# hukenovs/blackman_harris_win

Measured on AMD Instinct MI355X. Metric: window Gsamples/s (BH-7, N=2^26, 32-bit) + fraction of HBM-write roofline, higher is better.
Workload: dtype int64

## Files before the change

### blackman_harris_win_amd/csrc/bhw_build.hip

```cpp
#include "bhw_device.h"

namespace {

template <typename T>
__global__ __launch_bounds__(kBlock) void k_table_build(BhwCordicCfg cfg, uint32_t entries, void *__restrict__ table)
{
    __shared__ T lut_s[32];
    stage_lut<T>(cfg, lut_s);
    const uint32_t u = blockIdx.x * kBlock + threadIdx.x;
    if (u >= entries) return;
    T x, y;
    cordic_q1<T>(lut_s, (T)cfg.x0, (T)((T)u << cfg.z_shl), (int)cfg.n_iter, x, y);
    const int32_t c = (int32_t)(x >> cfg.out_shr), sn = (int32_t)(y >> cfg.out_shr);
    const int2 head = make_int2(__builtin_amdgcn_readfirstlane(c), __builtin_amdgcn_readfirstlane(sn));
    const int4 rec = cfg.tab_dlog > kPackLog ? reinterpret_cast<const int4 *>(cfg.tab_coarse)[u >> fmt_cell_log(cfg.tab_dlog)] : make_int4(0, 0, 0, 0);
    tab_store(table, u, cfg.phi_width - 2 - cfg.z_shr, cfg.tab_split, cfg.tab_dlog, const_cast<void *>(cfg.tab_coarse), c, sn, head, rec,
              cfg.tab_check);
}


template <int NITER, int FMT>
__global__ __launch_bounds__(kBuildThreads) void k_table_build_shared(BhwBuildPlan plan, void *__restrict__ table)
{
    __shared__ int64_t gx[kGroupsPerWg];
    __shared__ int64_t gy[kGroupsPerWg];
    __shared__ int32_t gz[kGroupsPerWg];
    __shared__ int32_t gk[kGroupsPerWg];
    __shared__ uint32_t lut_s[32];
    if (threadIdx.x < 32) lut_s[threadIdx.x] = plan.lut[threadIdx.x];
    __syncthreads();

    constexpr int n_iter = NITER;
    const uint32_t s = plan.z_shl;
    const uint32_t gpw = plan.groups_per_wg;
    const uint32_t group0 = blockIdx.x * gpw;
    const uint32_t n_groups = plan.entries >> 6;

    if (threadIdx.x < gpw) {
        const uint32_t g = group0 + threadIdx.x;
        const uint32_t u_first = g << 6;
        int64_t x = plan.x0, y = plan.x0;
        int32_t zf = (int32_t)((u_first << s) - lut_s[0]);
        const uint32_t span = 63u << s;
        int k = 1;
        bool live = g < n_groups;
        constexpr int kmax = n_iter < kPrefixMax ? n_iter : kPrefixMax;
#pragma unroll
        for (int kk = 1; kk < kmax; ++kk) {
            if (live) {
                const int32_t zl = (int32_t)((uint32_t)zf + span);
                if ((zf < 0) != (zl < 0)) {
                    live = false;
                } else {
                    rot_step(x, y, zf, kk, plan.lut[kk]);
                    k = kk + 1;
                }
            }
        }
        gx[threadIdx.x] = x;
        gy[threadIdx.x] = y;
        gz[threadIdx.x] = zf;
        gk[threadIdx.x] = k;
    }
    __syncthreads();

    const uint32_t wave = __builtin_amdgcn_readfirstlane(threadIdx.x >> 6), lane = threadIdx.x & 63u;
    uint32_t idx_a = lane, idx_m = 64u;
    if (plan.tab_split) {
        const uint32_t e = 1u << plan.log2_entries;
        if (lane & 1u)      { idx_a = (e >> 1) + (lane >> 1); idx_m = 32u; }
        else if (lane & 2u) { idx_a = (e >> 2) + (lane >> 2); idx_m = 16u; }
        else                { idx_a = lane >> 2;              idx_m = 16u; }
    }
    for (uint32_t gi = wave; gi < gpw; gi += kBuildThreads / 64) {
        const uint32_t g = __builtin_amdgcn_readfirstlane(group0 + gi);
        if (g >= n_groups) break;
        int64_t x = gx[gi], y = gy[gi];
        int32_t z = (int32_t)((uint32_t)gz[gi] + (lane << s));
        const int k0 = __builtin_amdgcn_readfirstlane(gk[gi]);
#pragma unroll
        for (int k = 1; k < NITER; ++k) {
            if (k >= kPrefixMax || k >= k0) rot_step(x, y, z, k, plan.lut[k]);
        }
        const int32_t c = (int32_t)(x >> plan.out_shr), sn = (int32_t)(y >> plan.out_shr);
        const int2 head = make_int2(__builtin_amdgcn_readfirstlane(c), __builtin_amdgcn_readfirstlane(sn));
        const uint32_t idx = idx_a + g * idx_m;
        if constexpr (FMT == 4) {
            const uint32_t u = (g << 6) + lane, nmask = 4u * plan.entries - 1u;
            int32_t *d_sin = reinterpret_cast<int32_t *>(table), *d_cos = reinterpret_cast<int32_t *>(const_cast<void *>(plan.tab_coarse));
#pragma unroll
            for (uint32_t q = 0; q < 4u; ++q) {
                int32_t oc, os;
                quadrant_map(q, c, sn, plan.pad0, oc, os);
                const uint32_t i = (q * plan.entries + u - plan.pad) & nmask;
                if (d_sin) d_sin[i] = os;
                if (d_cos) d_cos[i] = oc;
            }
        } else if constexpr (FMT == 0) {
            reinterpret_cast<int2 *>(table)[idx] = make_int2(c, sn);
        } else {
            static_assert(FMT == 1, "k_table_build_shared builds plain and delta16 tables (and the sin / cos sweep) only");
            const int32_t dc = c - head.x, ds = sn - head.y;
            if (plan.check_flag && !(fits_bits(dc, 16) && fits_bits(ds, 16))) atomicOr(plan.check_flag, 1u);
            reinterpret_cast<uint32_t *>(table)[idx] = ((uint32_t)dc & 0xFFFFu) | ((uint32_t)ds << 16);
            if (lane == 0u) reinterpret_cast<int2 *>(const_cast<void *>(plan.tab_coarse))[g] = head;
        }
    }
}

constexpr int kMirrorTail = 6;
constexpr int mirror_gpw(int threads) { return threads / 4; }
constexpr int mirror_heads_max(int threads) { return mirror_gpw(threads) / 2 + 8; }
constexpr int mirror_heads_pad(int threads) { return (mirror_heads_max(threads) + 63) / 64 * 64; }
constexpr int kTailZ = 256;

constexpr int kTailRows = 65;
struct TailD { int8_t v[kTailRows * 64 + 16]; };
constexpr TailD make_tail_d()
{
    TailD t{};
    for (int p = 0; p < 64; ++p)
        for (int v = 0; v < kTailRows; ++v) {
            int d = 0;
            for (int j = 0; j < kMirrorTail; ++j) d += ((p >> j) & 1) ? -(v >> j) : (v >> j);
            t.v[v * 64 + p] = (int8_t)d;
        }
    return t;
}
__device__ const TailD kTailD = make_tail_d();

constexpr int kRankSkip = 4;
constexpr int kRankCand = (1 << kRankSkip) + 1;
template <typename L>
__device__ __forceinline__ int32_t rank_threshold(uint32_t p, const L &l)
{
    int32_t t = 0;
#pragma unroll
    for (int m = 0; m + 1 < kRankSkip; ++m) {
        const uint32_t bit = 1u << (kRankSkip - 1 - m);
        if (p & (bit - 1u)) t += (p & bit) ? (int32_t)l[m] : -(int32_t)l[m];
    }
    return t;
}
template <int M, int R>
__device__ __forceinline__ void rank_candidates(uint32_t x, uint32_t y, uint32_t k, uint32_t bk, uint2 *out)
{
    if constexpr (M == kRankSkip) out[R] = make_uint2(x, y);
    else {
        const uint32_t a = y >> k, b = (x >> k) + bk;
        rank_candidates<M + 1, 2 * R>(x + a, y - b, k + 1u, bk >> 1, out);
        rank_candidates<M + 1, 2 * R + 1>(x - a, y + b, k + 1u, bk >> 1, out);
    }
}

template <int K, bool ZERO>
__device__ __forceinline__ void rot_narrow(uint32_t &x, uint32_t &y, int32_t &z, uint32_t &zacc, uint32_t lutk)
{
    uint32_t a, b;
    if constexpr (ZERO) {
        asm volatile("v_lshrrev_b32 %[a], %[k], %[y]\n\t"
                     "v_lshrrev_b32 %[b], %[k], %[x]\n\t"
                     "v_min_u32 %[za], %[za], %[z]\n\t"
                     "v_cmpx_gt_i32 vcc, 0, %[z]\n\t"
                     "v_add_u32 %[x], %[x], %[a]\n\t"
                     "v_sub_u32 %[y], %[y], %[b]\n\t"
                     "v_add_u32 %[z], %[z], %[l]\n\t"
                     "s_not_b64 exec, exec\n\t"
                     "v_sub_u32 %[x], %[x], %[a]\n\t"
                     "v_add_u32 %[y], %[y], %[b]\n\t"
                     "v_sub_u32 %[z], %[z], %[l]\n\t"
                     "s_mov_b64 exec, -1"
                     : [x] "+v"(x), [y] "+v"(y), [z] "+v"(z), [za] "+v"(zacc), [a] "=&v"(a), [b] "=&v"(b)
                     : [l] "s"(lutk), [k] "n"(K)
                     : "vcc", "scc");
    } else {
        asm volatile("v_lshrrev_b32 %[a], %[k], %[y]\n\t"
                     "v_lshrrev_b32 %[b], %[k], %[x]\n\t"
                     "v_cmpx_gt_i32 vcc, 0, %[z]\n\t"
                     "v_add_u32 %[x], %[x], %[a]\n\t"
                     "v_sub_u32 %[y], %[y], %[b]\n\t"
                     "v_add_u32 %[z], %[z], %[l]\n\t"
                     "s_not_b64 exec, exec\n\t"
                     "v_sub_u32 %[x], %[x], %[a]\n\t"
                     "v_add_u32 %[y], %[y], %[b]\n\t"
                     "v_sub_u32 %[z], %[z], %[l]\n\t"
                     "s_mov_b64 exec, -1"
                     : [x] "+v"(x), [y] "+v"(y), [z] "+v"(z), [a] "=&v"(a), [b] "=&v"(b)
                     : [l] "s"(lutk), [k] "n"(K)
                     : "vcc", "scc");
    }
}

template <int KA, int NITER>
__device__ __forceinline__ void rot_narrow_block(uint32_t &x, uint32_t &y, int32_t &z, uint32_t &zacc, const uint32_t (&l)[10], int e, uint32_t hi)
{
    uint32_t a, b;
#define BHW_ROT_I(lbl, i, HI_ADD)                                                                                       \
    #lbl ":\n\t"                                                                                                        \
    "v_lshrrev_b32 %[a], %[k" #i "], %[y]\n\t"                                                                          \
    "v_lshrrev_b32 %[b], %[k" #i "], %[x]\n\t"                                                                          \
    HI_ADD                                                                                                             \
    "v_min_u32 %[za], %[za], %[z]\n\t"                                                                                  \
    "v_cmpx_gt_i32 vcc, 0, %[z]\n\t"                                                                                    \
    "v_add_u32 %[x], %[x], %[a]\n\t"                                                                                    \
    "v_sub_u32 %[y], %[y], %[b]\n\t"                                                                                    \
    "v_add_u32 %[z], %[z], %[l" #i "]\n\t"                                                                              \
    "s_not_b64 exec, exec\n\t"                                                                                          \
    "v_sub_u32 %[x], %[x], %[a]\n\t"                                                                                    \
    "v_add_u32 %[y], %[y], %[b]\n\t"                                                                                    \
    "v_sub_u32 %[z], %[z], %[l" #i "]\n\t"                                                                              \
    "s_mov_b64 exec, -1\n"
#define BHW_ROT_PLAIN(i) BHW_ROT_I(i, i, "")
#define BHW_ROT_HI(i) BHW_ROT_I(2##i, i, "v_add_u32 %[b], %[c" #i "], %[b]\n\t")
#define BHW_ROT_DISPATCH(P, H)                                                                                         \
                 "s_cmp_gt_i32 %[e], 4\n\ts_cbranch_scc1 " #H "f\n\t"                                                 \
                 "s_cmp_lt_i32 %[e], 1\n\ts_cbranch_scc1 " #P "0f\n\t"                                                 \
                 "s_cmp_eq_u32 %[e], 1\n\ts_cbranch_scc1 " #P "1f\n\t"                                                 \
                 "s_cmp_eq_u32 %[e], 2\n\ts_cbranch_scc1 " #P "2f\n\t"                                                 \
                 "s_cmp_eq_u32 %[e], 3\n\ts_cbranch_scc1 " #P "3f\n\t"                                                 \
                 "s_branch " #P "4f\n"                                                                                  \
                 #H ":\n\t"                                                                                            \
                 "s_cmp_eq_u32 %[e], 5\n\ts_cbranch_scc1 " #P "5f\n\t"                                                 \
                 "s_cmp_eq_u32 %[e], 6\n\ts_cbranch_scc1 " #P "6f\n\t"                                                 \
                 "s_cmp_eq_u32 %[e], 7\n\ts_cbranch_scc1 " #P "7f\n\t"                                                 \
                 "s_cmp_eq_u32 %[e], 8\n\ts_cbranch_scc1 " #P "8f\n\t"                                                 \
                 "s_cmp_eq_u32 %[e], 9\n\ts_cbranch_scc1 " #P "9f\n\t"
    constexpr int S = NITER - 1 - KA;
    static_assert(S >= 9 && S <= 30, "bias shifts");
    asm volatile("s_cmp_lg_u32 %[hi], 0\n\ts_cbranch_scc1 100f\n\t"
                 BHW_ROT_DISPATCH(, 40)
                 "s_branch 10f\n"
                 BHW_ROT_PLAIN(0) BHW_ROT_PLAIN(1) BHW_ROT_PLAIN(2) BHW_ROT_PLAIN(3) BHW_ROT_PLAIN(4) BHW_ROT_PLAIN(5) BHW_ROT_PLAIN(6) BHW_ROT_PLAIN(7)
                 BHW_ROT_PLAIN(8) BHW_ROT_PLAIN(9)
                 "10:\n\ts_branch 200f\n"
                 "100:\n\t"
                 BHW_ROT_DISPATCH(2, 41)
                 "s_branch 200f\n"
                 BHW_ROT_HI(0) BHW_ROT_HI(1) BHW_ROT_HI(2) BHW_ROT_HI(3) BHW_ROT_HI(4) BHW_ROT_HI(5) BHW_ROT_HI(6) BHW_ROT_HI(7) BHW_ROT_HI(8) BHW_ROT_HI(9)
                 "200:"
                 : [x] "+v"(x), [y] "+v"(y), [z] "+v"(z), [za] "+v"(zacc), [a] "=&v"(a), [b] "=&v"(b)
                 : [e] "s"(e), [hi] "s"(hi), [l0] "s"(l[0]), [l1] "s"(l[1]), [l2] "s"(l[2]), [l3] "s"(l[3]), [l4] "s"(l[4]),
                   [l5] "s"(l[5]), [l6] "s"(l[6]), [l7] "s"(l[7]), [l8] "s"(l[8]), [l9] "s"(l[9]),
                   [k0] "n"(KA), [k1] "n"(KA + 1), [k2] "n"(KA + 2), [k3] "n"(KA + 3), [k4] "n"(KA + 4), [k5] "n"(KA + 5), [k6] "n"(KA + 6),
                   [k7] "n"(KA + 7), [k8] "n"(KA + 8), [k9] "n"(KA + 9),
                   [c0] "n"(1 << S), [c1] "n"(1 << (S - 1)), [c2] "n"(1 << (S - 2)), [c3] "n"(1 << (S - 3)), [c4] "n"(1 << (S - 4)),
                   [c5] "n"(1 << (S - 5)), [c6] "n"(1 << (S - 6)), [c7] "n"(1 << (S - 7)), [c8] "n"(1 << (S - 8)), [c9] "n"(1 << (S - 9))
                 : "vcc", "scc");
#undef BHW_ROT_I
#undef BHW_ROT_PLAIN
#undef BHW_ROT_HI
#undef BHW_ROT_DISPATCH
}

#ifdef BHW_BUILD_STAMPS
__device__ unsigned long long *g_build_stamps = nullptr;
#define BHW_STAMP(i) do { if (g_build_stamps && (threadIdx.x & 63u) == 0u) atomicMax(&g_build_stamps[blockIdx.x * 16u + (i)], (unsigned long long)wall_clock64()); } while (0)
#define BHW_STAMP_MIN(i) do { if (g_build_stamps && threadIdx.x == 0u) g_build_stamps[blockIdx.x * 16u + (i)] = (unsigned long long)wall_clock64(); } while (0)
#else
#define BHW_STAMP(i) do { } while (0)
#define BHW_STAMP_MIN(i) do { } while (0)
#endif

template <int BYTES>
__device__ __forceinline__ void table_store(void *__restrict__ table, uint32_t idx, uint32_t v)
{
    if constexpr (BYTES == 1) asm volatile("global_store_byte %0, %1, %2 sc1" :: "v"(idx), "v"(v), "s"(table) : "memory");
    else asm volatile("global_store_short %0, %1, %2 sc1" :: "v"(idx << 1), "v"(v), "s"(table) : "memory");
}

template <int NITER, int FMT, int THREADS>
__global__ __launch_bounds__(THREADS) __attribute__((amdgpu_waves_per_eu(8, 8))) void k_table_build_mirror(BhwBuildPlan plan, void *__restrict__ table)
{
    BHW_STAMP_MIN(0);
#ifdef BHW_BUILD_STAMPS
    if (g_build_stamps && threadIdx.x == 0u) {
        uint32_t hw, xcc;
        asm volatile("s_getreg_b32 %0, hwreg(HW_REG_HW_ID)\n\ts_getreg_b32 %1, hwreg(HW_REG_XCC_ID)" : "=s"(hw), "=s"(xcc));
        g_build_stamps[blockIdx.x * 16u + 6u] = hw;
        g_build_stamps[blockIdx.x * 16u + 7u] = xcc;
    }
#endif
    static_assert(FMT == 2 || FMT == 3 || FMT == 5, "residual / nibble entries");
    static_assert(NITER >= 21 && NITER <= 32, "narrow state: 32-bit words");
    static_assert(THREADS == 256 || THREADS == 1024, "workgroup shapes");
    constexpr uint32_t gpw = mirror_gpw(THREADS);
    constexpr uint32_t kHeads = mirror_heads_max(THREADS), kHeadsPad = mirror_heads_pad(THREADS);
    static_assert(gpw + 2 * kHeadsPad + 64 <= THREADS, "prefix lanes, two ranges of head chains, the tail-table wave");
    __shared__ int4 gst[gpw];
    __shared__ int2 ghi[gpw];
    __shared__ uint32_t lut_s[32];
    __shared__ uint8_t tail_p[2 * kTailZ];
    __shared__ __attribute__((aligned(16))) int8_t tail_d[kTailRows * 64 + 16];
    constexpr bool kRank = THREADS == 1024 || FMT != 5;
    __shared__ uint2 cand_s[kRank ? gpw * kRankCand : 1];
    __shared__ int2 rank_tab[kRank ? 8 << kRankSkip : 1];
    constexpr uint32_t kWorkMax = 8 * gpw;
    __shared__ uint32_t work_n;
    __shared__ uint32_t work_u[kWorkMax];
    __shared__ uint32_t esc_n;
    __shared__ int4 esc_list[FMT == 5 ? kEscFill : 1];
    __shared__ int4 esc_tab[FMT == 5 ? kEscSlots : 1];
    if (threadIdx.x < 32) lut_s[threadIdx.x] = plan.lut[threadIdx.x];
    if constexpr (FMT == 5) {
        if (threadIdx.x >= 64u && threadIdx.x < 64u + kEscSlots) esc_tab[threadIdx.x - 64u] = make_int4(-1, 0, 0, 0);
    }
#ifdef BHW_BUILD_STAMPS
    if (g_build_stamps && threadIdx.x == 0u) { asm volatile("s_waitcnt lgkmcnt(0)" ::: "memory"); g_build_stamps[blockIdx.x * 16u + 8u] = (unsigned long long)wall_clock64() | (plan.entries & 0u); }
#endif
    constexpr int n_iter = NITER;
    constexpr int KS = NITER - kMirrorTail;
    constexpr int KA = KS - 10;
    constexpr int kRankTop = KS - kRankSkip < kPrefixMax ? KS - kRankSkip : kPrefixMax;
    static_assert(kRankTop - KA < 8 && kRankTop + kRankSkip <= 31, "rank_tab rows; ROM words");
    const uint32_t s = plan.z_shl;
    const uint32_t group0 = blockIdx.x * gpw;
    const uint32_t E = plan.entries;
    const uint32_t n_groups = E >> 7;
    const uint32_t u_lo = group0 << 6;
    const uint32_t u_hi = ((group0 + gpw) << 6) < (n_groups << 6) ? ((group0 + gpw) << 6) : (n_groups << 6);
    const uint32_t m_last = (E >> 1) - 1u;
    if (threadIdx.x == 0) {
        work_n = 0u;
        esc_n = 0u;
        if (u_hi == (E >> 1)) {
            work_u[0] = E >> 1;
            work_n = 1u;
        }
    }
    if (threadIdx.x >= (uint32_t)THREADS - 64u) {
        const uint32_t t3 = threadIdx.x - ((uint32_t)THREADS - 64u);
#pragma unroll
        for (int q = 0; q < 5; ++q)
            if (t3 + 64u * q < (uint32_t)(kTailRows * 64 + 16) / 16u) reinterpret_cast<int4 *>(tail_d)[t3 + 64u * q] = reinterpret_cast<const int4 *>(kTailD.v)[t3 + 64u * q];
#pragma unroll
        for (int q = 0; q < 2 * kTailZ / 64; ++q) {
            const uint32_t zi = t3 + 64u * (uint32_t)q;
            int32_t z = (int32_t)zi - kTailZ;
            uint32_t p = 0u;
#pragma unroll
            for (int j = 0; j < kMirrorTail; ++j) {
                if (z < 0) { p |= 1u << j; z += (int32_t)plan.lut[KS + j]; } else z -= (int32_t)plan.lut[KS + j];
            }
            tail_p[zi] = (uint8_t)p;
        }
        if (kRank && t3 < (1u << kRankSkip)) {
#pragma unroll
            for (int row = 0; row <= kRankTop - KA; ++row) {
                const uint32_t l[kRankSkip] = {plan.lut[KA + row], plan.lut[KA + row + 1], plan.lut[KA + row + 2], plan.lut[KA + row + 3]};
                int32_t off = 0;
#pragma unroll
                for (int m = 0; m < kRankSkip; ++m) off += (t3 >> (kRankSkip - 1 - m)) & 1u ? (int32_t)l[m] : -(int32_t)l[m];
                rank_tab[(row << kRankSkip) + t3] = make_int2(off, t3 ? rank_threshold(t3, l) : INT32_MIN);
            }
        }
        BHW_STAMP(9);
    }


    __shared__ int32_t hc[2][kHeads], hs[2][kHeads];
    const uint32_t d = fmt_cell_log(plan.tab_dlog);
    const uint32_t cells_total = E >> d;
    uint32_t cell_lo[2] = {0u, 0u}, n_cell[2] = {0u, 0u}, r_lo[2] = {u_lo, 0u}, r_hi[2] = {u_hi, 0u};
    {
        const uint32_t a = u_lo > 1u ? u_lo : 1u, b = (u_hi - 1u) < m_last ? (u_hi - 1u) : m_last;
        if (a <= b) { r_lo[1] = E - b; r_hi[1] = E - a + 1u; }
        if (a <= b && b == (E >> 1) - 1u) r_lo[1] = E >> 1;
    }
#pragma unroll
    for (int w = 0; w < 2; ++w)
        if (r_hi[w] > r_lo[w]) {
            cell_lo[w] = r_lo[w] >> d;
            n_cell[w] = ((r_hi[w] - 1u) >> d) - cell_lo[w] + 1u;
        }
    if (threadIdx.x >= gpw && threadIdx.x < gpw + 2u * kHeadsPad) {
        const uint32_t w = (threadIdx.x - gpw) / kHeadsPad;
        const uint32_t t = (threadIdx.x - gpw) % kHeadsPad;
        if (n_cell[w] && t < n_cell[w] + 2u) {
            const int64_t cell = (t <= n_cell[w]) ? (int64_t)cell_lo[w] + t : (int64_t)cell_lo[w] - 1;
            if (cell >= 0 && cell < (int64_t)cells_total) {
                int64_t x = plan.x0, y = plan.x0;
                int32_t z = (int32_t)((((uint32_t)cell << d) << s) - plan.lut[0]);
#pragma unroll
                for (int r = 1; r < n_iter; ++r) rot_step(x, y, z, r, plan.lut[r]);
                hc[w][t] = (int32_t)(x >> plan.out_shr);
                hs[w][t] = (int32_t)(y >> plan.out_shr);
            }
        }
        BHW_STAMP(10);
    }

    constexpr int kcap = KS < kPrefixMax ? KS : kPrefixMax;
    if (threadIdx.x < gpw) {
        const uint32_t g = group0 + threadIdx.x;
        const uint32_t u_first = g << 6;
        int64_t x = plan.x0, y = plan.x0;
        int32_t zf = (int32_t)((u_first << s) - plan.lut[0]);
        const uint32_t span = 63u << s;
        int k = 1;
        bool live = g < n_groups;
        uint32_t zero0 = 0u;
#pragma unroll
        for (int kk = 1; kk < kcap; ++kk) {
            if (live) {
                const int32_t zl = (int32_t)((uint32_t)zf + span);
                if ((zf < 0) != (zl < 0)) {
                    live = false;
                } else {
                    zero0 |= (uint32_t)(zf == 0);
                    rot_step(x, y, zf, kk, plan.lut[kk]);
                    k = kk + 1;
                }
            }
        }
        const int64_t drift = ((int64_t)1 << (NITER - k + 1)) + 2, lim = (int64_t)1 << NITER;
        const bool narrow = x >= drift && y >= drift && x + drift < lim && y + drift < lim;
        constexpr int64_t kBias = (int64_t)1 << (NITER - 1);
        const bool hi = !narrow && k >= KS - 10 && y >= drift && y + drift < lim && x - kBias >= drift && x - kBias + drift < ((int64_t)1 << 32) &&
                        x + drift < lim + ((int64_t)1 << KS);
        const int64_t xp = hi ? x - kBias : x;
        uint32_t flags = zero0 | (narrow || hi ? 2u : 0u) | (hi ? 4u : 0u) | (g == 0u ? 8u : 0u);
        uint32_t w0 = (uint32_t)xp, w1 = (uint32_t)y, kw = (uint32_t)k;
        if (kRank && (narrow || hi) && k >= KA && k <= kRankTop) {
            uint32_t l[kRankSkip - 1] = {};
#pragma unroll
            for (int kk = KA; kk <= kRankTop; ++kk)
                if (k == kk) {
#pragma unroll
                    for (int m = 0; m + 1 < kRankSkip; ++m) l[m] = plan.lut[kk + m];
                }
            uint64_t mask = 0ull;
            uint32_t below = 0u, above = 0u;
            bool ok = true;
            int32_t prev = INT32_MIN;
            const int32_t round_up = (int32_t)((1u << s) - 1u) - zf;
#pragma unroll
            for (uint32_t p = 1; p < (1u << kRankSkip); ++p) {
                const int32_t t = rank_threshold(p, l);
                ok = ok && t > prev;
                prev = t;
                const int32_t first = (t + round_up) >> s;
                if (first <= 0) ++below;
                else if (first > 63) ++above;
                else mask |= 1ull << (first - 1);
            }
            if (ok && (uint32_t)__builtin_popcountll(mask) + below + above == (1u << kRankSkip) - 1u) {
                rank_candidates<0, 0>((uint32_t)xp, (uint32_t)y, (uint32_t)k, hi ? 1u << (NITER - 1 - k) : 0u, &cand_s[threadIdx.x * kRankCand]);
                w0 = (uint32_t)mask;
                w1 = (uint32_t)(mask >> 32);
                kw = (uint32_t)(k + kRankSkip) | (below << 16) | ((uint32_t)(k - KA) << (20 + kRankSkip + 3));
                flags |= 16u;
            }
        }
        gst[threadIdx.x] = make_int4((int32_t)w0, (int32_t)w1, zf, (int32_t)(kw | (flags << 8)));
        ghi[threadIdx.x] = make_int2((int32_t)(xp >> 32), (int32_t)(y >> 32));
        BHW_STAMP(11);
    }
    BHW_STAMP(1);
    __syncthreads();

    __shared__ int4 hrec[2][kHeads];
    {
        const uint32_t w = threadIdx.x / kHeadsPad, t = threadIdx.x % kHeadsPad;
        if (w < 2u && t < n_cell[w]) {
            const uint32_t cell = cell_lo[w] + t;
            int4 r;
            if (cell + 1u < cells_total) r = make_int4(hc[w][t], hs[w][t], hc[w][t + 1] - hc[w][t], hs[w][t + 1] - hs[w][t]);
            else {
                const uint32_t tp = t ? t - 1u : n_cell[w] + 1u;
                r = make_int4(hc[w][t], hs[w][t], hc[w][t] - hc[w][tp], hs[w][t] - hs[w][tp]);
            }
            if constexpr (FMT == 5) { r.x += (int32_t)kEscBias; r.y += (int32_t)kEscBias; }
            if constexpr (fmt_is_nibble(FMT)) { r.x -= 8; r.y -= 8; }
            hrec[w][t] = r;
            if constexpr (fmt_is_nibble(FMT)) { r.z *= 2; r.w *= 2; }
            if ((cell << d) >= r_lo[w])
                reinterpret_cast<int4 *>(const_cast<void *>(plan.tab_coarse))[cell] = r;
        }
    }
    __syncthreads();
    BHW_STAMP_MIN(2);
    auto record_of = [&](int w, uint32_t cell) -> int4 { return hrec[w][cell - cell_lo[w]]; };

    auto store_entry = [&](auto CHECKED, uint32_t idx, int32_t c, int32_t sn, const int4 rec, uint32_t pos) {
        if constexpr (FMT == 5) {
            const int2 p = tab_predict(rec, pos, d);
            const uint32_t nc = (uint32_t)(c - p.x), ns = (uint32_t)(sn - p.y);
            uint32_t v = nc | (ns << 4);
            if (__builtin_expect((int)(nc - 1u > 14u) | (int)(ns > 15u), 0)) {
                const uint32_t slot = atomicAdd(&esc_n, 1u);
                if (slot < kEscFill) esc_list[slot] = make_int4((int32_t)idx, c, sn, 0);
                v = kEscMarker;
            }
            table_store<1>(table, idx, v);
        } else if constexpr (FMT == 3) {
            const int2 p = tab_predict(rec, pos, d);
            const uint32_t nc = (uint32_t)(c - p.x), ns = (uint32_t)(sn - p.y);
            if constexpr (decltype(CHECKED)::value) {
                if (plan.check_flag && (nc | ns) > 15u) atomicOr(plan.check_flag, 1u);
            }
            table_store<1>(table, idx, nc | (ns << 4));
        } else {
            const int2 p = tab_predict(rec, pos, d);
            const int32_t dc = c - p.x, ds = sn - p.y;
            if constexpr (decltype(CHECKED)::value) {
                if (plan.check_flag && !(fits_bits(dc, 8) && fits_bits(ds, 8))) atomicOr(plan.check_flag, 1u);
            }
            table_store<2>(table, idx, ((uint32_t)dc & 0xFFu) | ((uint32_t)ds << 8));
        }
    };

    const uint32_t wave = __builtin_amdgcn_readfirstlane(threadIdx.x >> 6), lane = threadIdx.x & 63u;
    uint32_t idx_a, idx_m, idx_i;
    if (lane & 1u)      { idx_a = (E >> 1) + (lane >> 1); idx_m = 32u; idx_i = E + (E >> 1) - 1u; }
    else if (lane & 2u) { idx_a = (E >> 2) + (lane >> 2); idx_m = 16u; idx_i = (E >> 1) + (E >> 2) - 1u; }
    else                { idx_a = lane >> 2;              idx_m = 16u; idx_i = E >> 2; }
    if (!plan.tab_split) { idx_a = lane; idx_m = 64u; idx_i = E; }
    const uint32_t fmask = (1u << d) - 1u;
    constexpr uint32_t kWaves = THREADS / 64;
    static_assert(gpw == 16u * kWaves, "a wave walks 16 groups: four at each priority");
    constexpr bool kWholeCells = THREADS % (1 << 9) == 0;
    const uint32_t gi_end = group0 >= n_groups ? 0u : n_groups - group0 < gpw ? n_groups - group0 : gpw;
    const uint32_t zlane = lane << s;
    const uint32_t cell_step = ((uint32_t)THREADS >> d) << 4;
    static_assert(KA >= 5 && KA < kcap && KS - KA == 10, "ten-rotation block");
    uint32_t rom[10];
#pragma unroll
    for (int i = 0; i < 10; ++i) {
        rom[i] = __builtin_amdgcn_readfirstlane(lut_s[KA + i]);
        asm volatile("" : "+s"(rom[i]));
    }
    auto build_groups = [&](auto CHECKED) {
        uint32_t u = ((group0 + wave) << 6) + lane;
        uint32_t st_off = wave * (uint32_t)sizeof(int4);
        asm volatile("" : "+v"(st_off));
        uint32_t cand_off = wave * (uint32_t)(kRankCand * sizeof(uint2));
        asm volatile("" : "+v"(cand_off));
        uint32_t idx = idx_a + (group0 + wave) * idx_m;
        uint32_t off1, pos1, off2, pos2;
        auto cells_of = [&]() {
            const uint32_t um = E - u;
            pos1 = u & fmask;
            off1 = ((u >> d) - cell_lo[0]) << 4;
            pos2 = um & fmask;
            off2 = ((um >> d) - cell_lo[1]) << 4;
        };
        cells_of();
        uint32_t gi = wave;
#pragma unroll 1
        for (uint32_t quarter = 0; quarter < 4u; ++quarter) {
            if (quarter == 0u) __builtin_amdgcn_s_setprio(3);
            else if (quarter == 1u) __builtin_amdgcn_s_setprio(2);
            else if (quarter == 2u) __builtin_amdgcn_s_setprio(1);
            else __builtin_amdgcn_s_setprio(0);
            const uint32_t q_end = (quarter + 1u) * 4u * kWaves < gi_end ? (quarter + 1u) * 4u * kWaves : gi_end;
#pragma unroll 1
            for (; gi < q_end; gi += kWaves) {
                const int4 st = *reinterpret_cast<const int4 *>(reinterpret_cast<const char *>(gst) + st_off);
                const uint32_t kf = __builtin_amdgcn_readfirstlane((uint32_t)st.w);
                const int k0 = (int)(kf & 0xFFu);
                const uint32_t gf = (kf >> 8) & 0xFFu;
                int32_t z = (int32_t)((uint32_t)st.z + zlane);
                uint64_t zmask = 0ull;
                int32_t c1, s1, c2, s2;
                if (gf & 2u) {
                    uint32_t x = (uint32_t)st.x, y = (uint32_t)st.y;
                    uint32_t zacc = ~0u;
                    if (kRank && (gf & 16u)) {
                        const uint32_t rank = __builtin_amdgcn_mbcnt_hi((uint32_t)st.y, __builtin_amdgcn_mbcnt_lo((uint32_t)st.x, ((uint32_t)st.w >> 16) & 15u));
                        const uint2 cs = *reinterpret_cast<const uint2 *>(reinterpret_cast<const char *>(cand_s) + cand_off + (rank << 3));
                        const int2 rt = *reinterpret_cast<const int2 *>(reinterpret_cast<const char *>(rank_tab) + ((uint32_t)st.w >> 20) + (rank << 3));
                        zacc = (uint32_t)z - (uint32_t)rt.y;
                        z -= rt.x;
                        x = cs.x;
                        y = cs.y;
                    } else if (k0 < KA) {
#define BHW_NARROW(K) if constexpr (K < KA) { if (K >= k0) rot_narrow<K, true>(x, y, z, zacc, K < 9 ? (uint32_t)__builtin_amdgcn_readfirstlane(lut_s[K]) : plan.lut[K]); }
                        BHW_NARROW(1) BHW_NARROW(2) BHW_NARROW(3) BHW_NARROW(4) BHW_NARROW(5) BHW_NARROW(6) BHW_NARROW(7) BHW_NARROW(8)
                        BHW_NARROW(9) BHW_NARROW(10) BHW_NARROW(11) BHW_NARROW(12) BHW_NARROW(13) BHW_NARROW(14) BHW_NARROW(15)
#undef BHW_NARROW
                    }
                    const uint32_t hi = (gf >> 2) & 1u;
                    rot_narrow_block<KA, NITER>(x, y, z, zacc, rom, k0 - KA, hi);
                    zmask = __builtin_amdgcn_ballot_w64(zacc == 0u);
                    const uint32_t xrow6 = hi << (NITER - 1 - KS + 6);
                    const uint32_t bias_out = (hi << (NITER - 1)) >> plan.out_shr;
                    static_assert(KS <= 26, "unrolled to rotation 25");
                    constexpr uint32_t lowm = (1u << KS) - 1u;
                    const uint32_t zi = (uint32_t)(z + kTailZ);
                    const uint32_t mx = (x + 128u) & lowm, my = (y + 128u) & lowm;
                    const uint32_t unsafe = (uint32_t)((mx < my ? mx : my) < 256u) | (uint32_t)((zi - 1u) >= (uint32_t)(2 * kTailZ - 1));
                    if (__builtin_expect(__builtin_amdgcn_ballot_w64(unsafe != 0u) == 0ull, 1)) {
                        const uint32_t xx = ((x >> KS) << 6) + xrow6, yy = (y >> KS) << 6;
                        const uint32_t p1 = tail_p[zi], p2 = tail_p[2u * kTailZ - zi];
                        const int32_t dx1 = tail_d[p1 + yy], dy1 = tail_d[p1 + xx], dx2 = tail_d[p2 + xx], dy2 = tail_d[p2 + yy];
                        c1 = (int32_t)(((x - (uint32_t)dx1) >> plan.out_shr) + bias_out);
                        s1 = (int32_t)((y + (uint32_t)dy1) >> plan.out_shr);
                        c2 = (int32_t)((y - (uint32_t)dx2) >> plan.out_shr);
                        s2 = (int32_t)(((x + (uint32_t)dy2) >> plan.out_shr) + bias_out);
                    } else if (hi) {
                        int64_t xw = (int64_t)x + ((int64_t)1 << (NITER - 1)), yw = (int64_t)y;
                        int64_t x2 = yw, y2 = xw;
                        int32_t z2 = -z;
#pragma unroll 1
                        for (int k = KS; k < NITER; ++k) {
                            rot_step_dyn(xw, yw, z, k, lut_s[k], true);
                            rot_step_dyn(x2, y2, z2, k, lut_s[k], true);
                        }
                        c1 = (int32_t)(xw >> plan.out_shr); s1 = (int32_t)(yw >> plan.out_shr);
                        c2 = (int32_t)(x2 >> plan.out_shr); s2 = (int32_t)(y2 >> plan.out_shr);
                    } else {
                        uint32_t x2 = y, y2 = x;
                        int32_t z2 = -z;
                        uint32_t unused = 0u;
#define BHW_NARROW(K) if constexpr (K >= KS && K < NITER) { rot_narrow<K, false>(x, y, z, unused, plan.lut[K]); rot_narrow<K, false>(x2, y2, z2, unused, plan.lut[K]); }
                        BHW_NARROW(15) BHW_NARROW(16) BHW_NARROW(17) BHW_NARROW(18) BHW_NARROW(19) BHW_NARROW(20) BHW_NARROW(21) BHW_NARROW(22)
                        BHW_NARROW(23) BHW_NARROW(24) BHW_NARROW(25) BHW_NARROW(26) BHW_NARROW(27) BHW_NARROW(28) BHW_NARROW(29) BHW_NARROW(30)
                        BHW_NARROW(31)
#undef BHW_NARROW
                        c1 = (int32_t)(x >> plan.out_shr); s1 = (int32_t)(y >> plan.out_shr);
                        c2 = (int32_t)(x2 >> plan.out_shr); s2 = (int32_t)(y2 >> plan.out_shr);
                    }
                } else {
                    const int2 high = ghi[gi];
                    int64_t x = (int64_t)(((uint64_t)(uint32_t)high.x << 32) | (uint32_t)st.x), y = (int64_t)(((uint64_t)(uint32_t)high.y << 32) | (uint32_t)st.y);
#pragma unroll 1
                    for (int k = k0; k < KS; ++k) {
                        zmask |= __builtin_amdgcn_ballot_w64(z == 0);
                        rot_step_dyn(x, y, z, k, lut_s[k], k >= kMad24From);
                    }
                    int64_t x2 = y, y2 = x;
                    int32_t z2 = -z;
#pragma unroll 1
                    for (int k = KS; k < NITER; ++k) {
                        rot_step_dyn(x, y, z, k, lut_s[k], true);
                        rot_step_dyn(x2, y2, z2, k, lut_s[k], true);
                    }
                    c1 = (int32_t)(x >> plan.out_shr); s1 = (int32_t)(y >> plan.out_shr);
                    c2 = (int32_t)(x2 >> plan.out_shr); s2 = (int32_t)(y2 >> plan.out_shr);
                }
                const uint32_t own_idx = fmt_is_nibble(FMT) ? u : idx;
                store_entry(CHECKED, own_idx, c1, s1, *reinterpret_cast<const int4 *>(reinterpret_cast<const char *>(hrec[0]) + off1), pos1);
                auto store_image = [&]() {
                    store_entry(CHECKED, fmt_is_nibble(FMT) ? E - u : idx_i - idx, c2, s2,
                                *reinterpret_cast<const int4 *>(reinterpret_cast<const char *>(hrec[1]) + off2), pos2);
                };
                const uint32_t events = (uint32_t)zmask | (uint32_t)(zmask >> 32) | (gf & 9u);
                if (events == 0u) {
                    store_image();
                } else {
                    const bool replay = u != 0u && ((((zmask >> lane) & 1ull) != 0ull) || ((gf & 1u) && lane == 0u));
                    bool deferred = false;
                    if (replay) {
                        const uint32_t slot = atomicAdd(&work_n, 1u);
                        if (slot < kWorkMax) { work_u[slot] = u; deferred = true; }
                        else {
                            int64_t xf = plan.x0, yf = plan.x0;
                            int32_t zf = (int32_t)(((E - u) << s) - lut_s[0]);
#pragma unroll 1
                            for (int r = 1; r < n_iter; ++r) rot_step_dyn(xf, yf, zf, r, lut_s[r], r >= kMad24From);
                            c2 = (int32_t)(xf >> plan.out_shr);
                            s2 = (int32_t)(yf >> plan.out_shr);
                        }
                    }
                    if (u != 0u && !deferred) store_image();
                }
                u += (uint32_t)THREADS;
                st_off += kWaves * (uint32_t)sizeof(int4);
                cand_off += kWaves * (uint32_t)(kRankCand * sizeof(uint2));
                idx += kWaves * idx_m;
                if constexpr (kWholeCells) { off1 += cell_step; off2 -= cell_step; }
                else cells_of();
            }
        }
    };
    if constexpr (FMT == 5) build_groups(std::false_type{});
    else if (plan.check_flag) build_groups(std::true_type{});
    else build_groups(std::false_type{});
    BHW_STAMP_MIN(3);
    BHW_STAMP(4);
    __syncthreads();
    const uint32_t n_work = work_n < kWorkMax ? work_n : kWorkMax;
    for (uint32_t i = threadIdx.x; i < n_work; i += THREADS) {
        const uint32_t um = E - work_u[i];
        int64_t xf = plan.x0, yf = plan.x0;
        int32_t zf = (int32_t)((um << s) - plan.lut[0]);
#pragma unroll
        for (int r = 1; r < n_iter; ++r) rot_step(xf, yf, zf, r, plan.lut[r]);
        store_entry(std::true_type{}, tab_index(um, plan.log2_entries, plan.tab_split), (int32_t)(xf >> plan.out_shr), (int32_t)(yf >> plan.out_shr), record_of(1, um >> d), um & fmask);
    }
    if constexpr (FMT == 5) {
        __syncthreads();
        const uint32_t n_esc = esc_n < kEscFill ? esc_n : kEscFill;
        uint32_t tid = threadIdx.x;
        asm volatile("" : "+v"(tid));
        if (tid < n_esc) {
            const int4 it = esc_list[tid];
            uint32_t h = esc_slot((uint32_t)it.x);
#pragma unroll 1
            for (uint32_t i = 0; i < kEscSlots; ++i) {
                const uint32_t was = atomicCAS(reinterpret_cast<uint32_t *>(&esc_tab[h].x), ~0u, (uint32_t)it.x);
                if (was == ~0u || was == (uint32_t)it.x) { esc_tab[h].y = it.y; esc_tab[h].z = it.z; break; }
                h = (h + 1u) & (kEscSlots - 1u);
            }
        }
        __syncthreads();
        if (tid < kEscSlots) reinterpret_cast<int4 *>(plan.tab_esc)[(size_t)blockIdx.x * kEscSlots + tid] = esc_tab[tid];
        if (tid == 0u && esc_n > kEscFill && plan.check_flag) atomicOr(plan.check_flag, 1u);
    }
    BHW_STAMP(5);
}

template <int NITER>
__global__ __launch_bounds__(kBlock) void k_table_build_plain(BhwCordicCfg cfg, uint32_t entries, int2 *__restrict__ table)
{
    __shared__ uint32_t lut_s[32];
    if (threadIdx.x < 32) lut_s[threadIdx.x] = (uint32_t)cfg.lut[threadIdx.x];
    __syncthreads();
    const uint32_t u = blockIdx.x * kBlock + threadIdx.x;
    if (u >= entries) return;
    int64_t x = cfg.x0, y = cfg.x0;
    int32_t z = (int32_t)((u << cfg.z_shl) - lut_s[0]);
#pragma unroll
    for (int r = 1; r < NITER; ++r) rot_step(x, y, z, r, lut_s[r]);
    table[u] = make_int2((int32_t)(x >> cfg.out_shr), (int32_t)(y >> cfg.out_shr));
}

}


int bhwk_sincos_sweep(const BhwLaunch &l, const BhwCordicCfg &c, uint64_t theta0, int32_t *d_sin, int32_t *d_cos)
{
    hipStream_t st = (hipStream_t)l.stream;
    BhwBuildPlan plan;
    for (uint32_t k = 0; k < 32; ++k) plan.lut[k] = (uint32_t)c.lut[k];
    plan.entries = 1u << (c.phi_width - 2);
    plan.n_iter = c.n_iter;
    plan.z_shl = c.z_shl;
    plan.out_shr = c.out_shr;
    plan.log2_entries = c.phi_width - 2;
    plan.tab_split = 0;
    plan.tab_dlog = 0;
    plan.pad0 = c.ones_neg;
    plan.tab_coarse = d_cos;
    plan.x0 = c.x0;
    plan.check_flag = nullptr;
    plan.tab_esc = nullptr;
    const unsigned groups = plan.entries >> 6;
    plan.groups_per_wg = groups >= 64u * 1024u ? 64u : groups >= 16u * 1024u ? 16u : 4u;
    plan.pad = (uint32_t)(theta0 & ((1ull << c.phi_width) - 1ull));
    const dim3 grid((groups + plan.groups_per_wg - 1) / plan.groups_per_wg), block(kBuildThreads);
    if (!with_int_range<7, 32>(c.n_iter, [&](auto N) { launch(k_table_build_shared<N, 4>, grid, block, st, plan, (void *)d_sin); }))
        return (int)hipErrorInvalidValue;
    return finish(hipSuccess);
}

#ifdef BHW_BUILD_STAMPS
extern "C" int bhw_dbg_build_stamps(void *d_words)
{
    unsigned long long *p = (unsigned long long *)d_words;
    return (int)hipMemcpyToSymbol(HIP_SYMBOL(g_build_stamps), &p, sizeof p);
}
#endif

int bhwk_table_build(const BhwLaunch &l, const BhwCordicCfg &c_in, int32_t *d_table)
{
    const BhwCordicCfg c = table_layout(c_in);
    hipStream_t st = (hipStream_t)l.stream;
    const uint32_t entries = 1u << (c.phi_width - 2 - c.z_shr);
    const bool fits = (c.dat_width + c.out_shr <= 34);
    if (fits && c.n_iter >= 7 && entries < (1u << 20) && c.tab_dlog == 0 && !c.tab_split) {
        const dim3 grid(grid_for(entries)), block(kBlock);
        if (!with_int_range<7, 32>(c.n_iter, [&](auto N) { launch(k_table_build_plain<N>, grid, block, st, c, entries, (int2 *)d_table); }))
            return (int)hipErrorInvalidValue;
        return finish(hipSuccess);
    }
    if (entries >= 64 && fits && c.n_iter >= 2) {
        BhwBuildPlan plan;
        for (uint32_t k = 0; k < 32; ++k) plan.lut[k] = (uint32_t)c.lut[k];
        plan.entries = entries;
        plan.n_iter = c.n_iter;
        plan.z_shl = c.z_shl;
        plan.out_shr = c.out_shr;
        plan.log2_entries = c.phi_width - 2 - c.z_shr;
        plan.tab_split = c.tab_split;
        plan.tab_dlog = c.tab_dlog;
        plan.pad0 = 0;
        plan.tab_coarse = c.tab_coarse;
        plan.x0 = c.x0;
        plan.check_flag = c.tab_check;
        plan.tab_esc = const_cast<void *>(c.tab_esc);
        const unsigned groups = entries >> 6;
        plan.groups_per_wg = groups >= 64u * 1024u ? 64u : groups >= 16u * 1024u ? 16u : 4u;
        plan.pad = 0;
        const dim3 grid((groups + plan.groups_per_wg - 1) / plan.groups_per_wg), block(kBuildThreads);
        const int fmt = fmt_of(c.tab_dlog);
        if (c.n_iter < 21 && fmt != 0) return (int)hipErrorInvalidValue;
        if (bhwk_build_mirror_applies(c, entries)) {
            const unsigned own_groups = entries >> 7;
            const unsigned threads = bhwk_build_mirror_threads(entries);
            const unsigned mgpw = (unsigned)mirror_gpw((int)threads);
            const dim3 mgrid((own_groups + mgpw - 1) / mgpw), mblock(threads);
            plan.groups_per_wg = mgpw;
            const bool listed = with_int_range<21, 32>(c.n_iter, [&](auto N) {
                with_int_or_last<2, 3, 5>(fmt, [&](auto F) {
                    with_int_or_last<1024, 256>((int)threads, [&](auto T) {
                        launch(k_table_build_mirror<N, F, T>, mgrid, mblock, st, plan, (void *)d_table);
                    });
                });
            });
            return listed ? finish(hipSuccess) : (int)hipErrorInvalidValue;
        }
        if (fmt > 1) return (int)hipErrorInvalidValue;
        const bool listed = with_int_range<7, 32>(c.n_iter, [&](auto N) {
            if constexpr (N < 21) launch(k_table_build_shared<N, 0>, grid, block, st, plan, (void *)d_table);
            else with_int_or_last<0, 1>(fmt, [&](auto F) { launch(k_table_build_shared<N, F>, grid, block, st, plan, (void *)d_table); });
        });
        return listed ? finish(hipSuccess) : (int)hipErrorInvalidValue;
    }
    if (c.tab_dlog > kPackLog) return (int)hipErrorInvalidValue;
    if (c.wide) launch(k_table_build<int64_t>, dim3(grid_for(entries)), dim3(kBlock), st, c, entries, (void *)d_table);
    else        launch(k_table_build<int32_t>, dim3(grid_for(entries)), dim3(kBlock), st, c, entries, (void *)d_table);
    return finish(hipSuccess);
}
```

Measured before the change: 754.7.

## Defer replay-lane collection to a post-loop event scan with a rank fast path

```diff
diff --git a/blackman_harris_win_amd/csrc/bhw_build.hip b/blackman_harris_win_amd/csrc/bhw_build.hip
--- a/blackman_harris_win_amd/csrc/bhw_build.hip
+++ b/blackman_harris_win_amd/csrc/bhw_build.hip
@@ -297,6 +297,7 @@
     constexpr uint32_t kWorkMax = 8 * gpw;
     __shared__ uint32_t work_n;
     __shared__ uint32_t work_u[kWorkMax];
+    constexpr bool kEvents = FMT != 5;
     __shared__ uint32_t esc_n;
     __shared__ int4 esc_list[FMT == 5 ? kEscFill : 1];
     __shared__ int4 esc_tab[FMT == 5 ? kEscSlots : 1];
@@ -357,7 +358,11 @@
     }
 
 
-    __shared__ int32_t hc[2][kHeads], hs[2][kHeads];
+    __shared__ union { struct { int32_t c[2][kHeads], s[2][kHeads]; } h; uint64_t ev[gpw]; } heads_s;
+    static_assert(sizeof(heads_s.h) >= sizeof(heads_s.ev), "event words inside the head results");
+    auto &hc = heads_s.h.c;
+    auto &hs = heads_s.h.s;
+    auto &ev_s = heads_s.ev;
     const uint32_t d = fmt_cell_log(plan.tab_dlog);
     const uint32_t cells_total = E >> d;
     uint32_t cell_lo[2] = {0u, 0u}, n_cell[2] = {0u, 0u}, r_lo[2] = {u_lo, 0u}, r_hi[2] = {u_hi, 0u};
@@ -530,6 +535,7 @@
         asm volatile("" : "+s"(rom[i]));
     }
     auto build_groups = [&](auto CHECKED) {
+        constexpr bool kLate = kEvents && !decltype(CHECKED)::value;
         uint32_t u = ((group0 + wave) << 6) + lane;
         uint32_t st_off = wave * (uint32_t)sizeof(int4);
         asm volatile("" : "+v"(st_off));
@@ -562,25 +568,17 @@
                 int32_t z = (int32_t)((uint32_t)st.z + zlane);
                 uint64_t zmask = 0ull;
                 int32_t c1, s1, c2, s2;
-                if (gf & 2u) {
-                    uint32_t x = (uint32_t)st.x, y = (uint32_t)st.y;
-                    uint32_t zacc = ~0u;
-                    if (kRank && (gf & 16u)) {
-                        const uint32_t rank = __builtin_amdgcn_mbcnt_hi((uint32_t)st.y, __builtin_amdgcn_mbcnt_lo((uint32_t)st.x, ((uint32_t)st.w >> 16) & 15u));
-                        const uint2 cs = *reinterpret_cast<const uint2 *>(reinterpret_cast<const char *>(cand_s) + cand_off + (rank << 3));
-                        const int2 rt = *reinterpret_cast<const int2 *>(reinterpret_cast<const char *>(rank_tab) + ((uint32_t)st.w >> 20) + (rank << 3));
-                        zacc = (uint32_t)z - (uint32_t)rt.y;
-                        z -= rt.x;
-                        x = cs.x;
-                        y = cs.y;
-                    } else if (k0 < KA) {
-#define BHW_NARROW(K) if constexpr (K < KA) { if (K >= k0) rot_narrow<K, true>(x, y, z, zacc, K < 9 ? (uint32_t)__builtin_amdgcn_readfirstlane(lut_s[K]) : plan.lut[K]); }
-                        BHW_NARROW(1) BHW_NARROW(2) BHW_NARROW(3) BHW_NARROW(4) BHW_NARROW(5) BHW_NARROW(6) BHW_NARROW(7) BHW_NARROW(8)
-                        BHW_NARROW(9) BHW_NARROW(10) BHW_NARROW(11) BHW_NARROW(12) BHW_NARROW(13) BHW_NARROW(14) BHW_NARROW(15)
-#undef BHW_NARROW
-                    }
-                    const uint32_t hi = (gf >> 2) & 1u;
-                    rot_narrow_block<KA, NITER>(x, y, z, zacc, rom, k0 - KA, hi);
+                auto rank_entry = [&](uint32_t &x, uint32_t &y, uint32_t &zacc) {
+                    const uint32_t rank = __builtin_amdgcn_mbcnt_hi((uint32_t)st.y, __builtin_amdgcn_mbcnt_lo((uint32_t)st.x, ((uint32_t)st.w >> 16) & 15u));
+                    const uint2 cs = *reinterpret_cast<const uint2 *>(reinterpret_cast<const char *>(cand_s) + cand_off + (rank << 3));
+                    const int2 rt = *reinterpret_cast<const int2 *>(reinterpret_cast<const char *>(rank_tab) + ((uint32_t)st.w >> 20) + (rank << 3));
+                    zacc = (uint32_t)z - (uint32_t)rt.y;
+                    z -= rt.x;
+                    x = cs.x;
+                    y = cs.y;
+                };
+                auto narrow_finish = [&](uint32_t x, uint32_t y, uint32_t zacc, const int e, const uint32_t hi) {
+                    rot_narrow_block<KA, NITER>(x, y, z, zacc, rom, e, hi);
                     zmask = __builtin_amdgcn_ballot_w64(zacc == 0u);
                     const uint32_t xrow6 = hi << (NITER - 1 - KS + 6);
                     const uint32_t bias_out = (hi << (NITER - 1)) >> plan.out_shr;
@@ -620,6 +618,48 @@
                         c1 = (int32_t)(x >> plan.out_shr); s1 = (int32_t)(y >> plan.out_shr);
                         c2 = (int32_t)(x2 >> plan.out_shr); s2 = (int32_t)(y2 >> plan.out_shr);
                     }
+                };
+                auto store_own = [&]() {
+                    store_entry(CHECKED, fmt_is_nibble(FMT) ? u : idx, c1, s1, *reinterpret_cast<const int4 *>(reinterpret_cast<const char *>(hrec[0]) + off1), pos1);
+                };
+                auto store_image = [&]() {
+                    store_entry(CHECKED, fmt_is_nibble(FMT) ? E - u : idx_i - idx, c2, s2,
+                                *reinterpret_cast<const int4 *>(reinterpret_cast<const char *>(hrec[1]) + off2), pos2);
+                };
+                auto store_events = [&](uint64_t ev) {
+                    *reinterpret_cast<uint64_t *>(reinterpret_cast<char *>(ev_s) + (st_off >> 1)) = ev;
+                };
+                auto next_group = [&]() {
+                    u += (uint32_t)THREADS;
+                    st_off += kWaves * (uint32_t)sizeof(int4);
+                    cand_off += kWaves * (uint32_t)(kRankCand * sizeof(uint2));
+                    idx += kWaves * idx_m;
+                    if constexpr (kWholeCells) { off1 += cell_step; off2 -= cell_step; }
+                    else cells_of();
+                };
+                if constexpr (kLate) {
+                    if (__builtin_expect(gf == 18u, 1)) {
+                        uint32_t x, y, zacc;
+                        rank_entry(x, y, zacc);
+                        narrow_finish(x, y, zacc, k0 - KA, 0u);
+                        store_own();
+                        if (((zmask >> lane) & 1ull) == 0ull) store_image();
+                        store_events(zmask);
+                        next_group();
+                        continue;
+                    }
+                }
+                if (gf & 2u) {
+                    uint32_t x = (uint32_t)st.x, y = (uint32_t)st.y;
+                    uint32_t zacc = ~0u;
+                    if (kRank && (gf & 16u)) rank_entry(x, y, zacc);
+                    else if (k0 < KA) {
+#define BHW_NARROW(K) if constexpr (K < KA) { if (K >= k0) rot_narrow<K, true>(x, y, z, zacc, K < 9 ? (uint32_t)__builtin_amdgcn_readfirstlane(lut_s[K]) : plan.lut[K]); }
+                        BHW_NARROW(1) BHW_NARROW(2) BHW_NARROW(3) BHW_NARROW(4) BHW_NARROW(5) BHW_NARROW(6) BHW_NARROW(7) BHW_NARROW(8)
+                        BHW_NARROW(9) BHW_NARROW(10) BHW_NARROW(11) BHW_NARROW(12) BHW_NARROW(13) BHW_NARROW(14) BHW_NARROW(15)
+#undef BHW_NARROW
+                    }
+                    narrow_finish(x, y, zacc, k0 - KA, (gf >> 2) & 1u);
                 } else {
                     const int2 high = ghi[gi];
                     int64_t x = (int64_t)(((uint64_t)(uint32_t)high.x << 32) | (uint32_t)st.x), y = (int64_t)(((uint64_t)(uint32_t)high.y << 32) | (uint32_t)st.y);
@@ -638,38 +678,40 @@
                     c1 = (int32_t)(x >> plan.out_shr); s1 = (int32_t)(y >> plan.out_shr);
                     c2 = (int32_t)(x2 >> plan.out_shr); s2 = (int32_t)(y2 >> plan.out_shr);
                 }
-                const uint32_t own_idx = fmt_is_nibble(FMT) ? u : idx;
-                store_entry(CHECKED, own_idx, c1, s1, *reinterpret_cast<const int4 *>(reinterpret_cast<const char *>(hrec[0]) + off1), pos1);
-                auto store_image = [&]() {
-                    store_entry(CHECKED, fmt_is_nibble(FMT) ? E - u : idx_i - idx, c2, s2,
-                                *reinterpret_cast<const int4 *>(reinterpret_cast<const char *>(hrec[1]) + off2), pos2);
+                store_own();
+                auto image_or_defer = [&]() {
+                    const uint32_t events = (uint32_t)zmask | (uint32_t)(zmask >> 32) | (gf & 9u);
+                    if (events == 0u) {
+                        store_image();
+                    } else {
+                        const bool replay = u != 0u && ((((zmask >> lane) & 1ull) != 0ull) || ((gf & 1u) && lane == 0u));
+                        bool deferred = false;
+                        if (replay) {
+                            const uint32_t slot = atomicAdd(&work_n, 1u);
+                            if (slot < kWorkMax) { work_u[slot] = u; deferred = true; }
+                            else {
+                                int64_t xf = plan.x0, yf = plan.x0;
+                                int32_t zf = (int32_t)(((E - u) << s) - lut_s[0]);
+#pragma unroll 1
+                                for (int r = 1; r < n_iter; ++r) rot_step_dyn(xf, yf, zf, r, lut_s[r], r >= kMad24From);
+                                c2 = (int32_t)(xf >> plan.out_shr);
+                                s2 = (int32_t)(yf >> plan.out_shr);
+                            }
+                        }
+                        if (u != 0u && !deferred) store_image();
+                    }
                 };
-                const uint32_t events = (uint32_t)zmask | (uint32_t)(zmask >> 32) | (gf & 9u);
-                if (events == 0u) {
-                    store_image();
-                } else {
-                    const bool replay = u != 0u && ((((zmask >> lane) & 1ull) != 0ull) || ((gf & 1u) && lane == 0u));
-                    bool deferred = false;
-                    if (replay) {
-                        const uint32_t slot = atomicAdd(&work_n, 1u);
-                        if (slot < kWorkMax) { work_u[slot] = u; deferred = true; }
-                        else {
-                            int64_t xf = plan.x0, yf = plan.x0;
-                            int32_t zf = (int32_t)(((E - u) << s) - lut_s[0]);
-#pragma unroll 1
-                            for (int r = 1; r < n_iter; ++r) rot_step_dyn(xf, yf, zf, r, lut_s[r], r >= kMad24From);
-                            c2 = (int32_t)(xf >> plan.out_shr);
-                            s2 = (int32_t)(yf >> plan.out_shr);
-                        }
+                if constexpr (kLate) {
+                    if (__builtin_expect((gf & 8u) == 0u, 1)) {
+                        const uint64_t ev = zmask | (uint64_t)(gf & 1u);
+                        if (((ev >> lane) & 1ull) == 0ull) store_image();
+                        store_events(ev);
+                    } else {
+                        image_or_defer();
+                        store_events(0ull);
                     }
-                    if (u != 0u && !deferred) store_image();
-                }
-                u += (uint32_t)THREADS;
-                st_off += kWaves * (uint32_t)sizeof(int4);
-                cand_off += kWaves * (uint32_t)(kRankCand * sizeof(uint2));
-                idx += kWaves * idx_m;
-                if constexpr (kWholeCells) { off1 += cell_step; off2 -= cell_step; }
-                else cells_of();
+                } else image_or_defer();
+                next_group();
             }
         }
     };
@@ -679,6 +721,32 @@
     BHW_STAMP_MIN(3);
     BHW_STAMP(4);
     __syncthreads();
+    if constexpr (kEvents) {
+        if (!plan.check_flag) {
+            static_assert(gpw * 4u == (uint32_t)THREADS, "event scan: a quarter of a group's word per thread");
+            uint32_t bits = (threadIdx.x >> 2) < gi_end ? (uint32_t)(ev_s[threadIdx.x >> 2] >> ((threadIdx.x & 3u) << 4)) & 0xFFFFu : 0u;
+            if (bits) {
+                uint32_t slot = atomicAdd(&work_n, (uint32_t)__builtin_popcount(bits));
+                const uint32_t ub = ((group0 + (threadIdx.x >> 2)) << 6) + ((threadIdx.x & 3u) << 4);
+                do {
+                    const uint32_t ue = ub + (uint32_t)__builtin_ctz(bits);
+                    bits &= bits - 1u;
+                    if (slot < kWorkMax) work_u[slot] = ue;
+                    else {
+                        const uint32_t um = E - ue;
+                        int64_t xf = plan.x0, yf = plan.x0;
+                        int32_t zf = (int32_t)((um << s) - lut_s[0]);
+#pragma unroll 1
+                        for (int r = 1; r < n_iter; ++r) rot_step_dyn(xf, yf, zf, r, lut_s[r], r >= kMad24From);
+                        store_entry(std::false_type{}, tab_index(um, plan.log2_entries, plan.tab_split), (int32_t)(xf >> plan.out_shr), (int32_t)(yf >> plan.out_shr),
+                                    record_of(1, um >> d), um & fmask);
+                    }
+                    ++slot;
+                } while (bits);
+            }
+            __syncthreads();
+        }
+    }
     const uint32_t n_work = work_n < kWorkMax ? work_n : kWorkMax;
     for (uint32_t i = threadIdx.x; i < n_work; i += THREADS) {
         const uint32_t um = E - work_u[i];
```

Result: no change. 749.3 (-0.7%).
